# jasonppy/VoiceCraft

Measured on AMD Instinct MI355X. Metric: codec_tokens_per_sec, higher is better.
Workload: dtype bf16; 1 GPU; giga830M TTS, batch 1/GPU, Lx=80, 150 prompt frames -> 650 generated frames (16 s total), top_k=40, hipGraph=on; parallelism=dp1 (utterance-sharded, one all_gather)

## Files before the change

include/vc_engine.h:

```cpp
#ifndef VC_ENGINE_H
#define VC_ENGINE_H

#include <stdint.h>

#ifdef __cplusplus
extern "C" {
#endif

#define VC_OK 0
#define VC_EINVAL (-1)
#define VC_ESTATE (-2)
#define VC_EHIP (-3)
#define VC_ECAP (-4)
#define VC_EMISSING (-5)

#define VC_DTYPE_F32 0
#define VC_DTYPE_BF16 1
#define VC_DTYPE_I64 2

#define VC_MAX_CODEBOOKS 8
#define VC_MAX_SPANS 8
#define VC_MAX_SILENCE 8

typedef struct vc_engine vc_engine;
// ... 134 lines not shown
  void* x_out;
  int32_t dtype, H, hd, S_max, rows, nsplit, nt, fast, part16;
} vc_debug_attn_args;
int vc_debug_attn(const vc_debug_attn_args* a, void* stream);
typedef struct vc_debug_attn8_args {
  vc_debug_attn_args base;
  void* kcache8;
  void* vcache8;
  void* kvshift8;
  int32_t rps, pack;
} vc_debug_attn8_args;
int vc_debug_attn8(const vc_debug_attn8_args* a, void* stream);
int vc_kv8_quantize_host(const uint16_t* bf16_rows, int n_rows, int hd, uint8_t* codes, int8_t* shift);
int vc_box_probe(long long bytes, int hops, float res[2], void* stream);
int vc_debug_plan(const vc_model_cfg* cfg, int compute_dtype, int rows, int32_t out[16]);
int vc_debug_read(vc_engine* e, const char* name, void* host_dst, int64_t nbytes);
int vc_last_timing(const vc_engine* e, float ms[3]);
int vc_bench_kernel(vc_engine* e, const char* which, int n_rows, int iters, float* avg_ms,
                    double* alg_bytes, void* stream);

#ifdef __cplusplus
}
#endif
#endif
```

voicecraft_amd/_lib.py:

```python
from __future__ import annotations

import ctypes as C
import os
from pathlib import Path

HERE = Path(__file__).resolve().parent
LIB_PATH = HERE / "libvcengine.so"

VC_DTYPE_F32, VC_DTYPE_BF16, VC_DTYPE_I64 = 0, 1, 2
VC_MAX_SILENCE = 8


class ModelCfg(C.Structure):
    _fields_ = [(n, C.c_int32) for n in (
        "d_model", "nhead", "num_layers", "n_codebooks", "audio_vocab_size", "n_special", "text_rows",
        "head_hidden", "empty_token", "eog", "audio_pad_token", "eos", "reduced_eog", "encodec_sr",
        "max_n_spans", "max_seqs", "max_positions")]


class SampleCfg(C.Structure):
    _fields_ = [
        ("top_k", C.c_int32), ("top_p", C.c_float), ("temperature", C.c_float),
        ("stop_repetition", C.c_int32), ("n_silence", C.c_int32),
        ("silence_tokens", C.c_int32 * VC_MAX_SILENCE), ("seed", C.c_uint64),
# ... 67 lines not shown
    "vc_debug_sample": (C.c_int, [C.c_void_p, C.c_int, C.POINTER(SampleCfg), C.c_int, C.c_void_p, C.c_void_p]),
    "vc_debug_attn": (C.c_int, [C.POINTER(DebugAttnArgs), C.c_void_p]),
    "vc_debug_attn8": (C.c_int, [C.POINTER(DebugAttn8Args), C.c_void_p]),
    "vc_kv8_quantize_host": (C.c_int, [C.c_void_p, C.c_int, C.c_int, C.c_void_p, C.c_void_p]),
    "vc_edit": (C.c_int, [C.c_void_p, C.c_void_p, C.c_int, C.c_void_p, C.c_int, C.POINTER(C.c_int32), C.c_int,
                          C.POINTER(C.c_int32), C.POINTER(SampleCfg), C.c_void_p, C.c_int, C.c_void_p, C.c_int,
                          C.POINTER(C.c_int), C.c_void_p, C.c_int, C.POINTER(C.c_int), C.c_void_p]),
    "vc_edit_multi": (C.c_int, [C.c_void_p, C.c_int, C.c_void_p, C.POINTER(C.c_int32), C.c_void_p, C.POINTER(C.c_int32),
                                C.POINTER(C.c_int32), C.POINTER(C.c_int32), C.POINTER(C.c_int32), C.POINTER(SampleCfg),
                                C.c_void_p, C.c_int, C.c_void_p, C.c_int, C.POINTER(C.c_int), C.c_void_p, C.c_int,
                                C.POINTER(C.c_int), C.c_void_p]),
    "vc_pattern_shift": (C.c_int, [C.c_void_p, C.c_int, C.c_int, C.c_int, C.c_int64, C.c_void_p, C.c_void_p]),
    "vc_pattern_revert": (C.c_int, [C.c_void_p, C.c_int, C.c_int, C.c_int, C.c_int, C.c_int64, C.c_void_p, C.c_void_p]),
    "vc_pattern_unshift": (C.c_int, [C.c_void_p, C.c_int, C.c_int, C.c_void_p, C.c_void_p]),
    "vc_debug_plan": (C.c_int, [C.c_void_p, C.c_int, C.c_int, C.POINTER(C.c_int32)]),
    "vc_box_probe": (C.c_int, [C.c_longlong, C.c_int, C.POINTER(C.c_float), C.c_void_p]),
    "vc_debug_read": (C.c_int, [C.c_void_p, C.c_char_p, C.c_void_p, C.c_int64]),
    "vc_last_timing": (C.c_int, [C.c_void_p, C.POINTER(C.c_float)]),
    "vc_bench_kernel": (C.c_int, [C.c_void_p, C.c_char_p, C.c_int, C.c_int, C.POINTER(C.c_float),
                                  C.POINTER(C.c_double), C.c_void_p]),
}

_lib = None


def load() -> C.CDLL:
    global _lib
    if _lib is not None:
        return _lib
    path = Path(os.environ.get("VC_ENGINE_LIB", LIB_PATH))
# ... 29 lines not shown
```

voicecraft_amd/build.py:

```python
from __future__ import annotations

import hashlib
import os
import subprocess
import sys
from pathlib import Path

HERE = Path(__file__).resolve().parent
CSRC = HERE / "csrc"
LIB = HERE / "libvcengine.so"
SOURCES = ["vc_gemm.hip", "vc_gemm_pf.hip", "vc_gemm_wd.hip", "vc_gemm_w13.hip", "vc_gemm_w8.hip", "vc_attn.hip", "vc_tokens.hip", "vc_engine.hip", "vc_codec.hip"]
FLAGS = ["--offload-arch=gfx950", "-O3", "-std=c++17", "-fPIC", "-Wno-unused-result", "-Wno-unused-value"]


def _hipcc() -> str:
    for cand in (os.environ.get("HIPCC"), "/opt/rocm/bin/hipcc", "hipcc"):
        if cand and (os.path.isabs(cand) and os.path.exists(cand) or not os.path.isabs(cand)):
            return cand
    raise RuntimeError("hipcc not found")


def _digest(paths) -> str:
    h = hashlib.sha256()
    for p in sorted(paths):
        h.update(p.name.encode())
        h.update(p.read_bytes())
# ... 59 lines not shown
```

voicecraft_amd/csrc/vc_common.h:

```cpp
#pragma once
#include <hip/hip_runtime.h>
#include <stdint.h>
#include "../../include/vc_engine.h"

typedef __attribute__((ext_vector_type(4))) float f32x4;
typedef __attribute__((ext_vector_type(8))) __bf16 bf16x8;
typedef __attribute__((ext_vector_type(4))) unsigned int u32x4;

#define VC_ROWS 16
#define VC_MAX_SEQS 64
#ifndef VC_MAX_ROWS
#define VC_MAX_ROWS 2048
#endif
#define VC_SLAB_ROWS (VC_MAX_ROWS + 5)
#define VC_MAX_NSPLIT 8
#define VC_MAX_KSPLIT 4
#define VC_MAX_SEG 32
#ifndef VC_TH_QKV
#define VC_TH_QKV 12
#endif
#define VC_VPL 34

struct bf16_t { uint16_t u; };

// ... 354 lines not shown
hipError_t vc_launch_gemm_frp(const GemmArgs& a, int dtype, hipStream_t s);
int vc_gemm_frp_ok(int rows, int N, int K, int dtype);
hipError_t vc_launch_gemm_qp(const GemmArgs& a, int dtype, hipStream_t s);
int vc_gemm_qp_ok(int rows, int N, int K, int dtype);
enum { VC_PK_W13 = 0, VC_PK_W8 = 1, VC_PK_N = 2 };
struct vc_packed_kind {
  int group_frags, group_u4;
  int lc;
  hipError_t (*pack)(const uint4* img, long n_frags, uint4* planes, unsigned char* side, unsigned int* counts, hipStream_t s);
  hipError_t (*row)(const GemmArgs& a, const uint4* planes, const uint32_t* side, int pro, int epi, hipStream_t s);
};
const vc_packed_kind& vc_packed(int kind);
int vc_gemm_packed_fr1_ng(int kind, int N, int K, int dtype, int nw);
hipError_t vc_launch_w13_pack(const uint4* img, long n_frags, uint4* planes, unsigned char* side, unsigned int* counts, hipStream_t s);
hipError_t vc_launch_gemm_fr1_w13(const GemmArgs& a, const uint4* planes, const uint32_t* side, int pro, int epi, hipStream_t s);
hipError_t vc_launch_w8_pack(const uint4* img, long n_frags, uint4* planes, unsigned char* side, unsigned int* counts, hipStream_t s);
hipError_t vc_launch_gemm_fr1_w8(const GemmArgs& a, const uint4* planes, const uint32_t* side, int pro, int epi, hipStream_t s);
extern int vc_blk_dbg_mask;
enum { VC_LC_ROWS_GEMM = 0, VC_LC_MT2 = 1, VC_LC_MT4 = 2, VC_LC_BLK64 = 3, VC_LC_BLK128_SBS = 4, VC_LC_BLK128_2X2 = 5,
       VC_LC_BLK64_OCC2 = 6, VC_LC_LN_ROWS = 7, VC_LC_ROWS_ATTN = 8, VC_LC_TILE_ATTN = 9, VC_LC_ROWS_GEMM_FR = 10, VC_LC_BIG256 = 11, VC_LC_BIG128 = 12, VC_LC_ROW_GEMM_FR1 = 13, VC_LC_TILE_ATTN64 = 14, VC_LC_ROWS_GEMM_FRP = 15, VC_LC_WD = 16, VC_LC_ROWS_GEMM_QP = 17, VC_LC_W13 = 18, VC_LC_W8 = 19, VC_LC_KV8_ATTN = 20, VC_LC_KV8_PACK = 21, VC_LC_N = 22 };
extern long long vc_launch_counts[VC_LC_N];
hipError_t vc_launch_ln_rows(const GemmArgs& a, int dtype, hipStream_t s);
hipError_t vc_launch_attn(const AttnArgs& a, int dtype, int rows_cap, hipStream_t s);
hipError_t vc_launch_kv8_pack(const Kv8PackArgs& a, hipStream_t s);
hipError_t vc_launch_tile_attn(const AttnArgs& a, int dtype, hipStream_t s);
hipError_t vc_launch_tile_attn64(const AttnArgs& a, hipStream_t s);
hipError_t vc_launch_prompt(const PromptArgs& a, hipStream_t s);
hipError_t vc_launch_sample(const SampleArgs& a, bool grouped, hipStream_t s);
struct RepackArgs {
  SeqState* st;
  SeqState* st_fin;
  float* dec_h;
  int* row_seq;
  int* row_pos;
  int* logit_row;
// ... 92 lines not shown
```

voicecraft_amd/csrc/vc_engine.hip:

```cpp
#include <math.h>
#include <stdarg.h>
#include <stdio.h>
#include <stdlib.h>
#include <limits.h>
#include <string.h>

#include <algorithm>
#include <chrono>
#include <deque>
#include <map>
#include <string>
#include <tuple>
#include <vector>

#include "vc_common.h"

namespace {

std::string g_create_err;

struct RawTensor {
  std::vector<int64_t> shape;
  float* dev = nullptr;
  long numel = 0;
// ... 4 lines not shown
  uint4 *Wo8 = nullptr, *W28 = nullptr;
  uint4 *Wqkv16 = nullptr;
  uint4 *Wqkv8 = nullptr;
  float *bqkv = nullptr, *bo = nullptr, *b1 = nullptr, *b2 = nullptr;
  float bo_mean = 0.f, b2_mean = 0.f;
  float *wg_qkv = nullptr, *wg_1 = nullptr;
  void *kc = nullptr, *vc = nullptr;
  unsigned char *kc8 = nullptr, *vc8 = nullptr;
  signed char* sh8 = nullptr;
  struct Packed {
    uint4* planes = nullptr;
    uint32_t* side = nullptr;
    int state = 0;
    int refused = 0;
  } packed[VC_PK_N][2];
};
enum { W13_F2 = 0, W13_QKV = 1 };
constexpr int W8_BITS[2] = {1, 4};

struct Plan { int n_tiles, KT, ksplit, nchunk; };

enum { HF_ERR = 0, HF_STAGE = 1, HF_SHARE = 2, HF_ACTIVE = 8, HF_LIVE0 = 9, HF_LIVE1 = 10, HF_LIVE_STEPS = 11, HF_GATHER_N = 12 };
enum { HM_CAPTURE = 1, HM_INSTANTIATE = 2, HM_LOOP = 3, HM_SPARE = 4, HM_LAUNCHED = 5, HM_REPACKS = 6 };
enum { SS_ADMITTED = 0, SS_ADMITTED_LIVE = 1, SS_TURNS = 2, SS_WIDENINGS = 3, SS_NARROWINGS = 4, SS_LIVE_ROWS = 5, SS_LAUNCHED_ROWS = 6 };

}

struct vc_engine {
  vc_model_cfg cfg{};
  int device = 0;
// ... 54 lines not shown
  int attn_nt = 2;
  int fr_rows = VC_ROWS;
  int tile_attn = 2, tile_attn_min_rows = 768;
  int fr_one = 1;
  int fr_pair = 1;
  int qkv_p8 = 2;
  int qkv16 = 1;
  int wide_heads = 1;
  int wide_gemm = 1;
  int wd_stage = 1;
  int shrink = 1;
  bool has_fr8 = false, has_qkv8 = false, has_qkv16 = false;
  int w13 = 5;
  bool has_w13 = false;
  unsigned int* w13_counts = nullptr;
  int w8_req = 0;
  int w8 = 0;
  int kv8_req = 0;
  int kv8 = 0;
  Kv8Layer* kv8_tab = nullptr;
  int cur_rows = 0;
  int attn_fast = 1;
  int hq = 1;
  void *hqA = nullptr, *hqB = nullptr;
  float* row_mu[2] = {nullptr, nullptr};
  float* mu_zero = nullptr;
  int att_p16 = 1;
  static constexpr int attn_blocks_multi = 512, attn_blocks_one = 256;
  int prefill_rows_per_pass = VC_MAX_ROWS;
  hipEvent_t ev[3]{};
// ... 112 lines not shown
int pack_folded(vc_engine* e, const std::string& wkey, const std::string& bkey, const std::string& ln_prefix,
                int N, int Kdim, uint4** Wout, float** wg, float** cb, int th = 16) {
  const RawTensor *tw, *tb, *tg, *tbe;
  int rc;
  if ((rc = need(e, wkey, {N, Kdim}, &tw))) return rc;
  if ((rc = need(e, bkey, {N}, &tb))) return rc;
  if ((rc = need(e, ln_prefix + "weight", {Kdim}, &tg))) return rc;
  if ((rc = need(e, ln_prefix + "bias", {Kdim}, &tbe))) return rc;
  if ((rc = pack_matrix(e, wkey, N, Kdim, Wout, th, tg->dev))) return rc;
  if ((rc = dalloc(e, wg, (size_t)N))) return rc;
  if ((rc = dalloc(e, cb, (size_t)N))) return rc;
  HIPCHK(e, vc_launch_fold_vecs(tw->dev, tg->dev, tbe->dev, tb->dev, *wg, *cb, N, Kdim, e->dtype, 0));
  return VC_OK;
}

int pack_planes(vc_engine* e, Layer& ly, int kind, int which, const uint4* image, long n_frags) {
  if (!e->w13_counts) { int rc = dalloc(e, &e->w13_counts, (size_t)4); if (rc) return rc; }
  const vc_packed_kind& pk = vc_packed(kind);
  Layer::Packed& p = ly.packed[kind][which];
  const size_t mark = e->allocs.size();
  const double bytes0 = e->bytes_total;
  int rc;
  if ((rc = dalloc(e, &p.planes, (size_t)(n_frags / pk.group_frags) * pk.group_u4))) return rc;
  if ((rc = dalloc(e, &p.side, (size_t)(n_frags / 4)))) return rc;
  HIPCHK(e, pk.pack(image, n_frags, p.planes, reinterpret_cast<unsigned char*>(p.side), e->w13_counts, 0));
  unsigned int cnt[2] = {0, 0};
  HIPCHK(e, hipMemcpy(cnt, e->w13_counts, sizeof cnt, hipMemcpyDeviceToHost));
  p.refused = (int)cnt[0];
  if (cnt[0] == 0 && cnt[1] == 0) { p.state = 1; return VC_OK; }
  p.state = 2;
  while (e->allocs.size() > mark) { (void)hipFree(e->allocs.back()); e->allocs.pop_back(); }
  e->bytes_total = bytes0;
  p.planes = nullptr; p.side = nullptr;
  return VC_OK;
}

int keep_vec(vc_engine* e, const std::string& key, int n, float** out, float* mean = nullptr) {
  const RawTensor* t;
  int rc = need(e, key, {n}, &t);
  if (rc) return rc;
  rc = dalloc(e, out, (size_t)n);
  if (rc) return rc;
  HIPCHK(e, hipMemcpy(*out, t->dev, (size_t)n * 4, hipMemcpyDeviceToDevice));
  if (mean) {
    std::vector<float> host((size_t)n);
    HIPCHK(e, hipMemcpy(host.data(), t->dev, (size_t)n * 4, hipMemcpyDeviceToHost));
    double sum = 0.0;
    for (float v : host) sum += v;
    *mean = (float)(sum / n);
// ... 248 lines not shown
  GemmArgs g = base_args(e, rs, e->p_f1, 4 * d, d);
  g.Wp = ly.W1; nt_bit(e, g, NT_F1); g.bias = ly.b1; g.wg = ly.wg_1;
  g.out = e->act; g.out_ld = 4 * d; g.mt = p.mt;
  if (p.form == FORM_FR) {
    g.h_in = r.h_in;
    if (p.hq) {
      g.x_in = e->hqA; g.x_ld = d; g.row_mu = e->row_mu[1]; g.mu_shift = ly.bo_mean; g.row_mu_out = e->row_mu[0];
      HIPCHK(e, vc_launch_gemm(g, e->dtype, PRO_LNQ, EPI_RELU, 1, 1, s));
    } else {
      HIPCHK(e, vc_launch_gemm(g, e->dtype, PRO_LNW, EPI_RELU, 1, 1, s));
    }
    return VC_OK;
  }
  set_resid(e, g, r);
  if (!p.ln_launch) {
    HIPCHK(e, vc_launch_gemm(g, e->dtype, PRO_LN, EPI_RELU, 1, 1, s));
    return VC_OK;
  }
  g.x_in = e->xn; g.x_ld = d;
  if (p.wd) HIPCHK(e, vc_launch_gemm_wd(g, e->dtype, EPI_RELU, 1, 1, s));
  else HIPCHK(e, vc_launch_gemm(g, e->dtype, PRO_PLAIN, EPI_RELU, 1, 1, s));
  return VC_OK;
}

int site_ffn_down(vc_engine* e, const PassPlan& p, const RowSrc& rs, const Layer& ly, hipStream_t s) {
  const int d = e->d;
  GemmArgs g = base_args(e, rs, e->p_f2, d, 4 * d);
  g.x_in = e->act; g.x_ld = 4 * d;
  if (p.form == FORM_FR || p.fd) {
    g.Wp = ly.W28; g.bias = ly.b2;
    g.h_in = e->hA; g.h_out = e->hB;
// ... 421 lines not shown
}

int nonzero(int v) { return v ? 1 : 0; }
int two_or_one(int v) { return v == 2 ? 2 : 1; }
int low6(int v) { return v & 63; }
int whole_tiles(int v) { return v / VC_ROWS * VC_ROWS; }

struct Val { int vc_engine::*f; int lo, hi; };
struct OptDesc {
  const char *name, *env, *tag;
  Val v0;
  int (*pre)(int);
  Val v1;
  int (*check)(vc_engine*, const char* name, int v0);
  int vc_engine::*only_if;
};
using E = vc_engine;
const OptDesc OPTIONS[] = {
    {"graph_steps", "VC_GRAPH_STEPS", "g", {&E::steps_per_graph, 1, 64}},
    {"nt", "VC_NT", "nt", {&E::nt_decode, 0, 63}, low6, {&E::attn_nt, 0, 2}},
    {"finished_rows", "VC_FINISHED_ROWS", "fr", {&E::fr_rows, 0, VC_ROWS}, nullptr, {}, need_fr8},
    {"fr_pair", "VC_FR_PAIR", "fr", {&E::fr_pair, 0, 1}, nonzero},
    {"att_p16", "VC_ATT_P16", "fr", {&E::att_p16, 0, 1}, nonzero},
    {"hq", "VC_HQ", "fr", {&E::hq, 0, 1}, nonzero},
    {"tile_attn", "VC_TILE_ATTN", "ta", {&E::tile_attn, 1, 2}, two_or_one, {&E::tile_attn_min_rows, 64, INT_MAX}},
    {"fr_one", "VC_FR_ONE", "r1", {&E::fr_one, 0, 2}, nullptr, {}, need_fr8},
    {"attn_fast", "VC_ATTN_FAST", "r1", {&E::attn_fast, 0, 1}, nonzero},
    {"qkv_p8", "VC_QKV_P8", "r1", {&E::qkv_p8, 0, 2}, nullptr, {}, need_qkv8},
    {"qkv16", "VC_QKV16", "q16", {&E::qkv16, 0, 1}, nonzero, {}, need_qkv16},
    {"wide_heads", "VC_WIDE_HEADS", "q16", {&E::wide_heads, 0, 1}, nonzero},
    {"wide_gemm", "VC_WIDE_GEMM", "q16", {&E::wide_gemm, 0, 1}, nonzero},
    {"wd_stage", "VC_WD_STAGE", "q16", {&E::wd_stage, 0, 1}, nonzero},
    {"shrink", "VC_SHRINK", "sh", {&E::shrink, 0, 1}, nonzero},
    {"w13", "VC_W13", "w13", {&E::w13, 0, 5}, nullptr, {}, need_mask},
    {"w8", nullptr, "w8", {&E::w8, 0, 5}, nullptr, {}, need_w8, &E::w8_req},
    {"kv8", nullptr, "kv8", {&E::kv8, 0, 1}, nonzero, {}, need_kv8, &E::kv8_req},
    {"prefill_rows", "VC_PREFILL_ROWS", nullptr, {&E::prefill_rows_per_pass, VC_ROWS, VC_MAX_ROWS}, whole_tiles},
};

int apply_option(vc_engine* e, const std::string& name, const char* value) {
  int v[3] = {0, 0, 0};
  const int n = sscanf(value ? value : "", "%d,%d,%d", &v[0], &v[1], &v[2]);
  if (n < 1) return fail(e, VC_EINVAL, "option '%s': '%s' is not a number list", name.c_str(), value ? value : "(null)");
  for (const OptDesc& o : OPTIONS) {
    if (name != o.name) continue;
    if (o.check)
      if (const int rc = o.check(e, o.name, v[0])) return rc;
    e->*o.v0.f = std::max(o.v0.lo, std::min(o.pre ? o.pre(v[0]) : v[0], o.v0.hi));
    if (o.v1.f && n >= 2) e->*o.v1.f = std::max(o.v1.lo, std::min(v[1], o.v1.hi));
    return VC_OK;
  }
  return fail(e, VC_EINVAL, "unknown option '%s'", name.c_str());
}

void refresh_opt_state(vc_engine* e) {
  std::string& t = e->opt_state;
  t.clear();
  const char* tag = "";
  for (const OptDesc& o : OPTIONS) {
    if (!o.tag || (o.only_if && !(e->*o.only_if))) continue;
    if (strcmp(tag, o.tag)) t += std::string(t.empty() ? "" : "|") + o.tag + "=";
    else t += ",";
    tag = o.tag;
    t += std::to_string(e->*o.v0.f);
    if (o.v1.f) t += "," + std::to_string(e->*o.v1.f);
  }
}

int apply_env_presets(vc_engine* e) {
  for (const OptDesc& o : OPTIONS)
    if (const char* v = o.env ? getenv(o.env) : nullptr) {
      if (!strcmp(o.env, "VC_NT") && !strcmp(v, "1")) v = "63";
      if (const int rc = apply_option(e, o.name, v)) return rc;
    }
  refresh_opt_state(e);
// ... 24 lines not shown
  if (rows == 1) {
    out[8] = p.fd ? 1 : 0;
    out[9] = p.qkv_fr1 ? 1 : 0;
  }
  if (fr && rows <= VC_FR_MAX_ROWS) {
    out[10] = p.frp ? 1 : 0;
    out[9] = p.qp ? 2 : 0;
  }
  if (rows > VC_ROWS) {
    out[11] = p.wd ? 1 : 0;
    out[12] = wd_ksplit(&e, d, d); out[13] = wd_ksplit(&e, d, 4 * d);
    out[14] = vc_gemm_wd_kpw(d, compute_dtype, 1); out[15] = vc_gemm_wd_kpw(c->head_hidden, compute_dtype, 1);
  }
  return VC_OK;
}

extern "C" int vc_set_option(vc_engine* e, const char* name, const char* value) {
  int rc = check_idle(e);
  if (rc) return rc;
  if (!name || !value) return fail(e, VC_EINVAL, "null argument to vc_set_option");
  rc = apply_option(e, name, value);
  refresh_opt_state(e);
  return rc;
}

extern "C" const char* vc_version(void) { return "vcengine 0.1 (gfx950)"; }

extern "C" const char* vc_last_error(const vc_engine* e) { return e ? e->err.c_str() : g_create_err.c_str(); }

extern "C" int vc_create(const vc_model_cfg* c, int hip_device, vc_engine** out) {
// ... 147 lines not shown
void decide_images(vc_engine* e) {
  const int d = e->d;
  const char* env_fr = getenv("VC_FINISHED_ROWS");
  const char* env_f1 = getenv("VC_FR_ONE");
  const bool want_fr8 = !(env_fr && atoi(env_fr) == 0 && env_f1 && atoi(env_f1) == 0);
  const char* env_q16 = getenv("VC_QKV16");
  const bool want_qkv16 = env_q16 ? atoi(env_q16) != 0 : e->B_max > VC_ROWS;
  if (!want_qkv16) e->qkv16 = 0;
  const char* env_p8 = getenv("VC_QKV_P8");
  const bool want_p8 = !(env_p8 && atoi(env_p8) == 0) && !(env_f1 && atoi(env_f1) == 0);
  e->has_fr8 = want_fr8;
  e->has_qkv8 = want_fr8 && want_p8 && vc_gemm_fr1_ok(3 * d, d, e->dtype, 4);
  e->has_qkv16 = want_qkv16;
  const char* env_w13 = getenv("VC_W13");
  e->has_w13 = e->dtype == VC_DTYPE_BF16 && !(env_w13 && atoi(env_w13) == 0);
}

int pack_layer(vc_engine* e, int l) {
  const int d = e->d;
  const bool want_fr8 = e->has_fr8, want_qkv16 = e->has_qkv16;
  int rc;
  const std::string pre = "decoder.layers." + std::to_string(l) + ".";
  Layer& ly = e->layers[l];
  if ((rc = pack_folded(e, pre + "self_attn.in_proj_weight", pre + "self_attn.in_proj_bias", pre + "norm1.", 3 * d, d,
                        &ly.Wqkv, &ly.wg_qkv, &ly.bqkv, VC_TH_QKV))) return rc;
  if (want_qkv16) {
    const RawTensor* tg1;
    if ((rc = need(e, pre + "norm1.weight", {d}, &tg1))) return rc;
    if ((rc = pack_matrix(e, pre + "self_attn.in_proj_weight", 3 * d, d, &ly.Wqkv16, 16, tg1->dev))) return rc;
  }
// ... 3 lines not shown
                        &ly.W1, &ly.wg_1, &ly.b1))) return rc;
  if ((rc = pack_matrix(e, pre + "linear2.weight", d, 4 * d, &ly.W2))) return rc;
  if (want_fr8) {
    if ((rc = pack_matrix(e, pre + "self_attn.out_proj.weight", d, d, &ly.Wo8, VC_TH_RES))) return rc;
    if ((rc = pack_matrix(e, pre + "linear2.weight", d, 4 * d, &ly.W28, VC_TH_RES))) return rc;
    if (e->has_qkv8) {
      const RawTensor* tg1;
      if ((rc = need(e, pre + "norm1.weight", {d}, &tg1))) return rc;
      if ((rc = pack_matrix(e, pre + "self_attn.in_proj_weight", 3 * d, d, &ly.Wqkv8, VC_TH_RES, tg1->dev))) return rc;
    }
  }
  if ((rc = keep_vec(e, pre + "linear2.bias", d, &ly.b2, &ly.b2_mean))) return rc;
  const int pack_mask[VC_PK_N] = {e->has_w13 ? 5 : 0, e->w8_req};
  for (int kind = 0; kind < VC_PK_N; ++kind) {
    if ((pack_mask[kind] & W8_BITS[W13_F2]) && ly.W28 && vc_gemm_packed_fr1_ng(kind, d, 4 * d, e->dtype, VC_FR_WAVES) &&
        (rc = pack_planes(e, ly, kind, W13_F2, ly.W28, (long)(d / VC_TH_RES) * (4 * d / 64)))) return rc;
    if ((pack_mask[kind] & W8_BITS[W13_QKV]) && ly.Wqkv8 && vc_gemm_packed_fr1_ng(kind, 3 * d, d, e->dtype, 4) &&
        (rc = pack_planes(e, ly, kind, W13_QKV, ly.Wqkv8, (long)(3 * d / VC_TH_RES) * (d / 64)))) return rc;
  }
  const size_t cache_bytes = (size_t)e->B_max * e->H * e->S_max * e->hd * e->esz;
  if ((rc = dalloc(e, &ly.kc, cache_bytes))) return rc;
  if ((rc = dalloc(e, &ly.vc, cache_bytes))) return rc;
  if (e->kv8_req) {
    const size_t vals = (size_t)e->B_max * e->H * e->S_max * e->hd;
    if ((rc = dalloc0(e, &ly.kc8, vals, vals)) || (rc = dalloc0(e, &ly.vc8, vals, vals)) ||
        (rc = dalloc0(e, &ly.sh8, vals / e->hd * 2, vals / e->hd * 2))) return rc;
  }
  for (const char* k2 : {"self_attn.in_proj_weight", "self_attn.out_proj.weight", "linear1.weight", "linear2.weight"}) {
    auto it = e->raw.find(pre + k2);
    if (it != e->raw.end()) { HIPCHK(e, hipDeviceSynchronize()); (void)hipFree(it->second.dev); e->raw.erase(it); }
  }
  return VC_OK;
}

// ... 1618 lines not shown
  else if (n == "host_ms") { host_src = e->host_ms; avail = 8 * 8; }
  else if (n == "options") {
    memset(host_dst, 0, (size_t)nbytes);
    memcpy(host_dst, e->opt_state.c_str(), std::min<size_t>((size_t)nbytes > 0 ? (size_t)nbytes - 1 : 0, e->opt_state.size()));
    return VC_OK;
  }
  else if (n == "w13_stats" || n == "w8_stats") {
    const int kind = n == "w13_stats" ? VC_PK_W13 : VC_PK_W8;
    std::vector<int32_t> v;
    for (const Layer& ly : e->layers)
      for (int w = 0; w < 2; ++w) { v.push_back(ly.packed[kind][w].state); v.push_back(ly.packed[kind][w].refused); }
    if (nbytes > (int64_t)(v.size() * 4)) return fail(e, VC_ECAP, "debug buffer '%s' holds %lld bytes", n.c_str(), (long long)(v.size() * 4));
    memcpy(host_dst, v.data(), (size_t)nbytes);
    return VC_OK;
  }
  else if (n == "launch_counts") { host_src = vc_launch_counts; avail = VC_LC_N * 8; }
  else if (n == "stream") {
    if (!e->ts) return fail(e, VC_ESTATE, "no streaming TTS call is open (vc_tts_stream_begin)");
    if (nbytes != 3 * 4) return fail(e, VC_ECAP, "debug buffer 'stream' holds 12 bytes");
    const int32_t v[3] = {1 + e->ts->L.complete, e->ts->emitted, e->ts->L.over ? 1 : 0};
    memcpy(host_dst, v, sizeof v);
    return VC_OK;
  }
  else if (n == "session_slots") {
    if (!e->sess) return fail(e, VC_ESTATE, "no decode session is open (vc_session_open)");
    std::vector<int32_t> v{e->sess->B};
    v.insert(v.end(), e->sess->slot_ticket.begin(), e->sess->slot_ticket.end());
    if (nbytes != (int64_t)(v.size() * 4)) return fail(e, VC_ECAP, "debug buffer 'session_slots' holds %lld bytes", (long long)(v.size() * 4));
    memcpy(host_dst, v.data(), (size_t)nbytes);
    return VC_OK;
// ... 125 lines not shown
```

voicecraft_amd/engine.py:

```python
from __future__ import annotations

import ast
import ctypes as C
import logging
import math
import random
from argparse import Namespace
from typing import Iterable

import torch

from . import _lib
from ._lib import EngineError, ModelCfg, SampleCfg, check

_DTYPES = {"bf16": _lib.VC_DTYPE_BF16, "bfloat16": _lib.VC_DTYPE_BF16, torch.bfloat16: _lib.VC_DTYPE_BF16,
           "fp32": _lib.VC_DTYPE_F32, "float32": _lib.VC_DTYPE_F32, torch.float32: _lib.VC_DTYPE_F32}


def _sine_table(n: int, d: int) -> torch.Tensor:
    pos = torch.arange(0, n, dtype=torch.float32).unsqueeze(1)
    div = torch.exp(torch.arange(0, d, 2, dtype=torch.float32) * -(math.log(10000.0) / d))
    pe = torch.zeros(n, d)
    pe[:, 0::2] = torch.sin(pos * div)
    pe[:, 1::2] = torch.cos(pos * div)
# ... 554 lines not shown
        return bytes(self.debug_read("options", (256,), torch.uint8).tolist()).split(b"\0")[0].decode()

    def last_timing_ms(self):
        ms = (C.c_float * 3)()
        check(self.lib.vc_last_timing(self._h, ms), self._h, "vc_last_timing")
        return {"prefill_ms": ms[0], "decode_ms": ms[1], "total_ms": ms[2]}

    def bench_kernel(self, which: str, n_rows: int = 1, iters: int = 50):
        ms, nbytes = C.c_float(0), C.c_double(0)
        check(self.lib.vc_bench_kernel(self._h, which.encode(), n_rows, iters, C.byref(ms), C.byref(nbytes), self._stream()),
              self._h, "vc_bench_kernel")
        return ms.value, nbytes.value

    LAUNCH_FORMS = ("rows_gemm", "mt2", "mt4", "blk64", "blk128_sbs", "blk128_2x2", "blk64_occ2", "ln_rows", "rows_attn",
                    "tile_attn", "rows_gemm_fr", "big256", "big128", "row_gemm_fr1", "tile_attn64", "rows_gemm_frp", "wd", "rows_gemm_qp", "w13", "w8",
                    "kv8_attn", "kv8_pack")

    def launch_counts(self) -> dict:
        c = self.debug_read("launch_counts", (len(self.LAUNCH_FORMS),), torch.int64)
        return {n: int(c[i]) for i, n in enumerate(self.LAUNCH_FORMS)}

    W13_MATRICES = ("ffn_down", "qkv")
    W13_STATES = ("not_applicable", "packed", "refused")

    def w13_stats(self) -> list:
        L = int(self.args.num_decoder_layers)
        v = self.debug_read("w13_stats", (L, 2, 2), torch.int32).tolist()
        return [{m: {"state": self.W13_STATES[v[l][i][0]], "refused_fragments": v[l][i][1]} for i, m in enumerate(self.W13_MATRICES)}
                for l in range(L)]

    W8_MATRICES = ("ffn_down", "qkv")
    W8_MASK = 5

    def w8_stats(self) -> list:
        L = int(self.args.num_decoder_layers)
        v = self.debug_read("w8_stats", (L, 2, 2), torch.int32).tolist()
        return [{m: {"state": self.W13_STATES[v[l][i][0]], "refused_fragments": v[l][i][1]} for i, m in enumerate(self.W8_MATRICES)}
                for l in range(L)]

    def debug_read(self, name: str, shape, dtype=torch.float32) -> torch.Tensor:
        out = torch.empty(shape, dtype=dtype)
        check(self.lib.vc_debug_read(self._h, name.encode(), C.c_void_p(out.data_ptr()), out.numel() * out.element_size()),
              self._h, "vc_debug_read")
        return out
# ... 456 lines not shown
```

Before: 8004 codec-tokens/s.

## Add W13-packed single-row FFN up-projection kernel with fused LayerNorm prologue

Adds a new decode kernel for the FFN up-projection (linear1) that reads weights from the compressed W13 packed-plane format instead of dense bf16. The LayerNorm, residual-part summation and ReLU epilogue are fused in. Weights are packed at load time with norm2 folded in, and the dense image is freed afterwards. The aim is to cut HBM weight traffic for the memory-bound single-row GEMM. In exchange it adds a decode step and extra packing memory, and depends on the W13 compression being acceptable for this matrix.

```diff
diff --git a/include/vc_engine.h b/include/vc_engine.h
--- a/include/vc_engine.h
+++ b/include/vc_engine.h
@@ -172,6 +172,7 @@
 int vc_kv8_quantize_host(const uint16_t* bf16_rows, int n_rows, int hd, uint8_t* codes, int8_t* shift);
 int vc_box_probe(long long bytes, int hops, float res[2], void* stream);
 int vc_debug_plan(const vc_model_cfg* cfg, int compute_dtype, int rows, int32_t out[16]);
+int vc_debug_up13_tiles(int d_model, int compute_dtype);
 int vc_debug_read(vc_engine* e, const char* name, void* host_dst, int64_t nbytes);
 int vc_last_timing(const vc_engine* e, float ms[3]);
 int vc_bench_kernel(vc_engine* e, const char* which, int n_rows, int iters, float* avg_ms,
diff --git a/voicecraft_amd/_lib.py b/voicecraft_amd/_lib.py
--- a/voicecraft_amd/_lib.py
+++ b/voicecraft_amd/_lib.py
@@ -105,6 +105,7 @@
     "vc_pattern_revert": (C.c_int, [C.c_void_p, C.c_int, C.c_int, C.c_int, C.c_int, C.c_int64, C.c_void_p, C.c_void_p]),
     "vc_pattern_unshift": (C.c_int, [C.c_void_p, C.c_int, C.c_int, C.c_void_p, C.c_void_p]),
     "vc_debug_plan": (C.c_int, [C.c_void_p, C.c_int, C.c_int, C.POINTER(C.c_int32)]),
+    "vc_debug_up13_tiles": (C.c_int, [C.c_int, C.c_int]),
     "vc_box_probe": (C.c_int, [C.c_longlong, C.c_int, C.POINTER(C.c_float), C.c_void_p]),
     "vc_debug_read": (C.c_int, [C.c_void_p, C.c_char_p, C.c_void_p, C.c_int64]),
     "vc_last_timing": (C.c_int, [C.c_void_p, C.POINTER(C.c_float)]),
diff --git a/voicecraft_amd/build.py b/voicecraft_amd/build.py
--- a/voicecraft_amd/build.py
+++ b/voicecraft_amd/build.py
@@ -9,7 +9,7 @@
 HERE = Path(__file__).resolve().parent
 CSRC = HERE / "csrc"
 LIB = HERE / "libvcengine.so"
-SOURCES = ["vc_gemm.hip", "vc_gemm_pf.hip", "vc_gemm_wd.hip", "vc_gemm_w13.hip", "vc_gemm_w8.hip", "vc_attn.hip", "vc_tokens.hip", "vc_engine.hip", "vc_codec.hip"]
+SOURCES = ["vc_gemm.hip", "vc_gemm_pf.hip", "vc_gemm_wd.hip", "vc_gemm_w13.hip", "vc_gemm_w8.hip", "vc_gemm_up1.hip", "vc_attn.hip", "vc_tokens.hip", "vc_engine.hip", "vc_codec.hip"]
 FLAGS = ["--offload-arch=gfx950", "-O3", "-std=c++17", "-fPIC", "-Wno-unused-result", "-Wno-unused-value"]
 
 
diff --git a/voicecraft_amd/csrc/vc_common.h b/voicecraft_amd/csrc/vc_common.h
--- a/voicecraft_amd/csrc/vc_common.h
+++ b/voicecraft_amd/csrc/vc_common.h
@@ -392,11 +392,13 @@
 int vc_gemm_packed_fr1_ng(int kind, int N, int K, int dtype, int nw);
 hipError_t vc_launch_w13_pack(const uint4* img, long n_frags, uint4* planes, unsigned char* side, unsigned int* counts, hipStream_t s);
 hipError_t vc_launch_gemm_fr1_w13(const GemmArgs& a, const uint4* planes, const uint32_t* side, int pro, int epi, hipStream_t s);
+int vc_gemm_up1_ok(int d, int dtype);
+hipError_t vc_launch_gemm_up1(const GemmArgs& a, const uint4* planes, const uint32_t* side, hipStream_t s);
 hipError_t vc_launch_w8_pack(const uint4* img, long n_frags, uint4* planes, unsigned char* side, unsigned int* counts, hipStream_t s);
 hipError_t vc_launch_gemm_fr1_w8(const GemmArgs& a, const uint4* planes, const uint32_t* side, int pro, int epi, hipStream_t s);
 extern int vc_blk_dbg_mask;
 enum { VC_LC_ROWS_GEMM = 0, VC_LC_MT2 = 1, VC_LC_MT4 = 2, VC_LC_BLK64 = 3, VC_LC_BLK128_SBS = 4, VC_LC_BLK128_2X2 = 5,
-       VC_LC_BLK64_OCC2 = 6, VC_LC_LN_ROWS = 7, VC_LC_ROWS_ATTN = 8, VC_LC_TILE_ATTN = 9, VC_LC_ROWS_GEMM_FR = 10, VC_LC_BIG256 = 11, VC_LC_BIG128 = 12, VC_LC_ROW_GEMM_FR1 = 13, VC_LC_TILE_ATTN64 = 14, VC_LC_ROWS_GEMM_FRP = 15, VC_LC_WD = 16, VC_LC_ROWS_GEMM_QP = 17, VC_LC_W13 = 18, VC_LC_W8 = 19, VC_LC_KV8_ATTN = 20, VC_LC_KV8_PACK = 21, VC_LC_N = 22 };
+       VC_LC_BLK64_OCC2 = 6, VC_LC_LN_ROWS = 7, VC_LC_ROWS_ATTN = 8, VC_LC_TILE_ATTN = 9, VC_LC_ROWS_GEMM_FR = 10, VC_LC_BIG256 = 11, VC_LC_BIG128 = 12, VC_LC_ROW_GEMM_FR1 = 13, VC_LC_TILE_ATTN64 = 14, VC_LC_ROWS_GEMM_FRP = 15, VC_LC_WD = 16, VC_LC_ROWS_GEMM_QP = 17, VC_LC_W13 = 18, VC_LC_W8 = 19, VC_LC_KV8_ATTN = 20, VC_LC_KV8_PACK = 21, VC_LC_ROW_GEMM_UP1 = 22, VC_LC_N = 23 };
 extern long long vc_launch_counts[VC_LC_N];
 hipError_t vc_launch_ln_rows(const GemmArgs& a, int dtype, hipStream_t s);
 hipError_t vc_launch_attn(const AttnArgs& a, int dtype, int rows_cap, hipStream_t s);
diff --git a/voicecraft_amd/csrc/vc_engine.hip b/voicecraft_amd/csrc/vc_engine.hip
--- a/voicecraft_amd/csrc/vc_engine.hip
+++ b/voicecraft_amd/csrc/vc_engine.hip
@@ -42,6 +42,7 @@
     int state = 0;
     int refused = 0;
   } packed[VC_PK_N][2];
+  Packed up13;
 };
 enum { W13_F2 = 0, W13_QKV = 1 };
 constexpr int W8_BITS[2] = {1, 4};
@@ -126,6 +127,8 @@
   int w13 = 5;
   bool has_w13 = false;
   unsigned int* w13_counts = nullptr;
+  int up13 = 1;
+  bool has_up13 = false;
   int w8_req = 0;
   int w8 = 0;
   int kv8_req = 0;
@@ -268,10 +271,9 @@
   return VC_OK;
 }
 
-int pack_planes(vc_engine* e, Layer& ly, int kind, int which, const uint4* image, long n_frags) {
+int pack_planes(vc_engine* e, Layer::Packed& p, int kind, const uint4* image, long n_frags) {
   if (!e->w13_counts) { int rc = dalloc(e, &e->w13_counts, (size_t)4); if (rc) return rc; }
   const vc_packed_kind& pk = vc_packed(kind);
-  Layer::Packed& p = ly.packed[kind][which];
   const size_t mark = e->allocs.size();
   const double bytes0 = e->bytes_total;
   int rc;
@@ -287,6 +289,27 @@
   e->bytes_total = bytes0;
   p.planes = nullptr; p.side = nullptr;
   return VC_OK;
+}
+
+void dfree(vc_engine* e, void* p, size_t bytes) {
+  auto it = std::find(e->allocs.begin(), e->allocs.end(), p);
+  if (it == e->allocs.end()) return;
+  e->allocs.erase(it);
+  (void)hipFree(p);
+  e->bytes_total -= (double)bytes;
+}
+
+int pack_up13(vc_engine* e, Layer& ly, const std::string& pre) {
+  const int d = e->d;
+  const RawTensor* tg2;
+  uint4* img = nullptr;
+  int rc;
+  if ((rc = need(e, pre + "norm2.weight", {d}, &tg2))) return rc;
+  if ((rc = pack_matrix(e, pre + "linear1.weight", 4 * d, d, &img, VC_TH_RES, tg2->dev))) return rc;
+  const long n_frags = (long)(4 * d / VC_TH_RES) * (d / 64);
+  rc = pack_planes(e, ly.up13, VC_PK_W13, img, n_frags);
+  dfree(e, img, (size_t)n_frags * 1024);
+  return rc;
 }
 
 int keep_vec(vc_engine* e, const std::string& key, int n, float** out, float* mean = nullptr) {
@@ -565,7 +588,9 @@
   }
   set_resid(e, g, r);
   if (!p.ln_launch) {
-    HIPCHK(e, vc_launch_gemm(g, e->dtype, PRO_LN, EPI_RELU, 1, 1, s));
+    const bool up1 = p.fd && e->up13 && ly.up13.state == 1 && g.nt && r.n_parts >= 1 && r.n_parts <= 2;
+    if (up1) HIPCHK(e, vc_launch_gemm_up1(g, ly.up13.planes, ly.up13.side, s));
+    else HIPCHK(e, vc_launch_gemm(g, e->dtype, PRO_LN, EPI_RELU, 1, 1, s));
     return VC_OK;
   }
   g.x_in = e->xn; g.x_ld = d;
@@ -1017,6 +1042,7 @@
   Val v1;
   int (*check)(vc_engine*, const char* name, int v0);
   int vc_engine::*only_if;
+  int quiet_at = -1;
 };
 using E = vc_engine;
 const OptDesc OPTIONS[] = {
@@ -1038,6 +1064,7 @@
     {"w13", "VC_W13", "w13", {&E::w13, 0, 5}, nullptr, {}, need_mask},
     {"w8", nullptr, "w8", {&E::w8, 0, 5}, nullptr, {}, need_w8, &E::w8_req},
     {"kv8", nullptr, "kv8", {&E::kv8, 0, 1}, nonzero, {}, need_kv8, &E::kv8_req},
+    {"up13", "VC_UP13", "up13", {&E::up13, 0, 1}, nonzero, {}, nullptr, nullptr, 1},
     {"prefill_rows", "VC_PREFILL_ROWS", nullptr, {&E::prefill_rows_per_pass, VC_ROWS, VC_MAX_ROWS}, whole_tiles},
 };
 
@@ -1061,7 +1088,7 @@
   t.clear();
   const char* tag = "";
   for (const OptDesc& o : OPTIONS) {
-    if (!o.tag || (o.only_if && !(e->*o.only_if))) continue;
+    if (!o.tag || (o.only_if && !(e->*o.only_if)) || (o.quiet_at >= 0 && e->*o.v0.f == o.quiet_at)) continue;
     if (strcmp(tag, o.tag)) t += std::string(t.empty() ? "" : "|") + o.tag + "=";
     else t += ",";
     tag = o.tag;
@@ -1116,6 +1143,8 @@
   }
   return VC_OK;
 }
+
+extern "C" int vc_debug_up13_tiles(int d_model, int compute_dtype) { return vc_gemm_up1_ok(d_model, compute_dtype); }
 
 extern "C" int vc_set_option(vc_engine* e, const char* name, const char* value) {
   int rc = check_idle(e);
@@ -1293,6 +1322,8 @@
   e->has_qkv16 = want_qkv16;
   const char* env_w13 = getenv("VC_W13");
   e->has_w13 = e->dtype == VC_DTYPE_BF16 && !(env_w13 && atoi(env_w13) == 0);
+  const char* env_up13 = getenv("VC_UP13");
+  e->has_up13 = want_fr8 && vc_gemm_up1_ok(d, e->dtype) != 0 && !(env_up13 && atoi(env_up13) == 0);
 }
 
 int pack_layer(vc_engine* e, int l) {
@@ -1326,10 +1357,11 @@
   const int pack_mask[VC_PK_N] = {e->has_w13 ? 5 : 0, e->w8_req};
   for (int kind = 0; kind < VC_PK_N; ++kind) {
     if ((pack_mask[kind] & W8_BITS[W13_F2]) && ly.W28 && vc_gemm_packed_fr1_ng(kind, d, 4 * d, e->dtype, VC_FR_WAVES) &&
-        (rc = pack_planes(e, ly, kind, W13_F2, ly.W28, (long)(d / VC_TH_RES) * (4 * d / 64)))) return rc;
+        (rc = pack_planes(e, ly.packed[kind][W13_F2], kind, ly.W28, (long)(d / VC_TH_RES) * (4 * d / 64)))) return rc;
     if ((pack_mask[kind] & W8_BITS[W13_QKV]) && ly.Wqkv8 && vc_gemm_packed_fr1_ng(kind, 3 * d, d, e->dtype, 4) &&
-        (rc = pack_planes(e, ly, kind, W13_QKV, ly.Wqkv8, (long)(3 * d / VC_TH_RES) * (d / 64)))) return rc;
-  }
+        (rc = pack_planes(e, ly.packed[kind][W13_QKV], kind, ly.Wqkv8, (long)(3 * d / VC_TH_RES) * (d / 64)))) return rc;
+  }
+  if (e->has_up13 && (rc = pack_up13(e, ly, pre))) return rc;
   const size_t cache_bytes = (size_t)e->B_max * e->H * e->S_max * e->hd * e->esz;
   if ((rc = dalloc(e, &ly.kc, cache_bytes))) return rc;
   if ((rc = dalloc(e, &ly.vc, cache_bytes))) return rc;
@@ -2978,6 +3010,13 @@
     memcpy(host_dst, v.data(), (size_t)nbytes);
     return VC_OK;
   }
+  else if (n == "up13_stats") {
+    std::vector<int32_t> v;
+    for (const Layer& ly : e->layers) { v.push_back(ly.up13.state); v.push_back(ly.up13.refused); }
+    if (nbytes > (int64_t)(v.size() * 4)) return fail(e, VC_ECAP, "debug buffer '%s' holds %lld bytes", n.c_str(), (long long)(v.size() * 4));
+    memcpy(host_dst, v.data(), (size_t)nbytes);
+    return VC_OK;
+  }
   else if (n == "launch_counts") { host_src = vc_launch_counts; avail = VC_LC_N * 8; }
   else if (n == "stream") {
     if (!e->ts) return fail(e, VC_ESTATE, "no streaming TTS call is open (vc_tts_stream_begin)");
diff --git a/voicecraft_amd/csrc/vc_gemm_up1.hip b/voicecraft_amd/csrc/vc_gemm_up1.hip
--- /dev/null
+++ b/voicecraft_amd/csrc/vc_gemm_up1.hip
@@ -0,0 +1,194 @@
+#include "vc_gemm_fr1.h"
+#include "vc_w13.h"
+
+struct Up1Args : Fr1PackedArgs {};
+
+int vc_gemm_up1_ok(int d, int dtype) {
+  if (dtype != VC_DTYPE_BF16 || d <= 0 || d % 1024 != 0) return 0;
+  const int ng = d / 1024, tiles = 4 * d / VC_TH_RES;
+  if (ng != 1 && ng != 2) return 0;
+  return tiles % 2 == 0 ? 2 : 0;
+}
+
+template <int F>
+__device__ __forceinline__ uint4 up1_frag(const uint4& la, const uint4& lb, const uint4& nb, uint32_t sg, uint32_t sidew) {
+  const uint32_t bm1 = vc_w13_bm1((sidew >> (8 * F)) & 0xffu);
+  const uint32_t l0 = F == 0 ? la.x : F == 1 ? la.z : F == 2 ? lb.x : lb.z;
+  const uint32_t l1 = F == 0 ? la.y : F == 1 ? la.w : F == 2 ? lb.y : lb.w;
+  const uint32_t n = F == 0 ? nb.x : F == 1 ? nb.y : F == 2 ? nb.z : nb.w;
+  uint4 w;
+  vc_w13_decode_half(l0, n, sg, 2 * F, bm1, &w.x, &w.y);
+  vc_w13_decode_half(l1, n, sg, 2 * F + 1, bm1, &w.z, &w.w);
+  return w;
+}
+
+template <int NG, int T>
+__global__ __launch_bounds__(256 * T) void row_gemm_up1_w13_k(const Up1Args wa) {
+  using WT = bf16_t;
+  using Tr = WTr<WT>;
+  constexpr int NW = 4, NPW = 4 * NG, TH = VC_TH_RES, SPT = 4 * TH;
+  constexpr int D = 1024 * NG, NQ = D / 4;
+  constexpr bool ON1 = NQ > 256;
+  const GemmArgs& a = wa.g;
+  extern __shared__ __attribute__((aligned(16))) char smem[];
+  VC_KTS_DECL();
+  VC_KTS(0);
+  const int tid = threadIdx.x, lane = tid & 63;
+  const int wv = __builtin_amdgcn_readfirstlane(tid >> 6);
+  const int wave = wv & 3, tg = wv >> 2;
+  const int nt = (int)blockIdx.x * T + tg;
+  const int m = lane & 15, kg = lane >> 4;
+  char* xl = smem;
+  f32x4* red = reinterpret_cast<f32x4*>(smem + (size_t)D * sizeof(WT)) + tg * (NW * 4);
+  float* stat = reinterpret_cast<float*>(smem + (size_t)D * sizeof(WT) + (size_t)T * NW * 4 * sizeof(f32x4));
+  float* msum = stat + 8;
+  const bool pro = wv < 4;
+
+  const int c0 = tid * 4, c1 = ON1 ? (tid + 256) * 4 : 0;
+  float4 pb0 = make_float4(0.f, 0.f, 0.f, 0.f), pb1 = pb0, x0 = pb0, x1 = pb0, p00 = pb0, p01 = pb0, p10 = pb0, p11 = pb0;
+  if (pro) {
+    pb0 = *reinterpret_cast<const float4*>(a.prev_bias + c0);
+    if constexpr (ON1) pb1 = *reinterpret_cast<const float4*>(a.prev_bias + c1);
+    x0 = *reinterpret_cast<const float4*>(a.h_in + c0);
+    if constexpr (ON1) x1 = *reinterpret_cast<const float4*>(a.h_in + c1);
+    const float* s0 = a.parts;
+    const float* s1 = a.parts + (long)a.rows_cap * D;
+    p00 = *reinterpret_cast<const float4*>(s0 + c0);
+    if constexpr (ON1) p10 = *reinterpret_cast<const float4*>(s0 + c1);
+    p01 = *reinterpret_cast<const float4*>(s1 + c0);
+    if constexpr (ON1) p11 = *reinterpret_cast<const float4*>(s1 + c1);
+  }
+
+  const int wunit = (m >> 3) * SPT + kg * TH + (m & 7);
+  const long G0 = ((long)nt * NW + wave) * NG;
+  const uint4* gbase = wa.planes + G0 * VC_W13_GROUP_U4;
+  uint4 la[NG], lb[NG], nb[NG];
+  uint32_t sg[NG], sb[NG];
+  int active = 1;
+#pragma unroll
+  for (int g = 0; g < NG; ++g) {
+    const uint4* gp = gbase + g * VC_W13_GROUP_U4;
+    la[g] = __builtin_bit_cast(uint4, __builtin_nontemporal_load(reinterpret_cast<const u32x4*>(gp + wunit)));
+    lb[g] = __builtin_bit_cast(uint4, __builtin_nontemporal_load(reinterpret_cast<const u32x4*>(gp + 64 + wunit)));
+    nb[g] = __builtin_bit_cast(uint4, __builtin_nontemporal_load(reinterpret_cast<const u32x4*>(gp + 128 + wunit)));
+    sg[g] = __builtin_nontemporal_load(reinterpret_cast<const uint32_t*>(gp + 192) + wunit);
+    __builtin_amdgcn_sched_barrier(0);
+    if (g == 0) {
+#pragma unroll
+      for (int j = 0; j < NG; ++j) sb[j] = wa.side[G0 + j];
+      active = *a.n_active;
+      __builtin_amdgcn_sched_barrier(0);
+    }
+  }
+  const int nfin = nt * TH + 4 * (lane & 1);
+  const float4 eb = *reinterpret_cast<const float4*>(a.bias + nfin);
+  const float4 ewg = *reinterpret_cast<const float4*>(a.wg + nfin);
+  __builtin_amdgcn_sched_barrier(0);
+#pragma unroll
+  for (int g = 0; g < NG; ++g) asm volatile("" : "+s"(sb[g]));
+  if (active == 0) return;
+  VC_KTS(1);
+
+  if (pro) {
+    if (a.has_prev_bias != 0) {
+      x0.x += pb0.x; x0.y += pb0.y; x0.z += pb0.z; x0.w += pb0.w;
+      x1.x += pb1.x; x1.y += pb1.y; x1.z += pb1.z; x1.w += pb1.w;
+    }
+    {
+      const bool u_ = 0 < a.n_parts;
+      x0.x += u_ ? p00.x : 0.f; x0.y += u_ ? p00.y : 0.f; x0.z += u_ ? p00.z : 0.f; x0.w += u_ ? p00.w : 0.f;
+      x1.x += u_ ? p10.x : 0.f; x1.y += u_ ? p10.y : 0.f; x1.z += u_ ? p10.z : 0.f; x1.w += u_ ? p10.w : 0.f;
+    }
+    {
+      const bool u_ = 1 < a.n_parts;
+      x0.x += u_ ? p01.x : 0.f; x0.y += u_ ? p01.y : 0.f; x0.z += u_ ? p01.z : 0.f; x0.w += u_ ? p01.w : 0.f;
+      x1.x += u_ ? p11.x : 0.f; x1.y += u_ ? p11.y : 0.f; x1.z += u_ ? p11.z : 0.f; x1.w += u_ ? p11.w : 0.f;
+    }
+    if (a.h_out && blockIdx.x == 0) {
+      *reinterpret_cast<float4*>(a.h_out + c0) = x0;
+      if constexpr (ON1) *reinterpret_cast<float4*>(a.h_out + c1) = x1;
+    }
+    float t_ = ((x0.x + x0.y) + (x0.z + x0.w)) + (ON1 ? ((x1.x + x1.y) + (x1.z + x1.w)) : 0.f);
+    t_ = wave_sum(t_);
+    if (lane == 0) msum[wave] = t_;
+  }
+  __syncthreads();
+  if (pro) {
+    const float4 ms_ = *reinterpret_cast<const float4*>(msum);
+    const float mu_ = ((ms_.x + ms_.y) + (ms_.z + ms_.w)) * (1.0f / (float)D);
+    WT* xr_ = reinterpret_cast<WT*>(xl);
+    float s1_ = 0.f, s2_ = 0.f;
+    {
+      const f32x4 y_ = {x0.x - mu_, x0.y - mu_, x0.z - mu_, x0.w - mu_};
+      const f32x4 q_ = store4r(xr_ + c0, y_);
+      s1_ += (q_[0] + q_[1]) + (q_[2] + q_[3]);
+      s2_ += (q_[0] * q_[0] + q_[1] * q_[1]) + (q_[2] * q_[2] + q_[3] * q_[3]);
+    }
+    if constexpr (ON1) {
+      const f32x4 y_ = {x1.x - mu_, x1.y - mu_, x1.z - mu_, x1.w - mu_};
+      const f32x4 q_ = store4r(xr_ + c1, y_);
+      s1_ += (q_[0] + q_[1]) + (q_[2] + q_[3]);
+      s2_ += (q_[0] * q_[0] + q_[1] * q_[1]) + (q_[2] * q_[2] + q_[3] * q_[3]);
+    }
+    s1_ = wave_sum(s1_);
+    s2_ = wave_sum(s2_);
+    if (lane == 0) { stat[wave * 2] = s1_; stat[wave * 2 + 1] = s2_; }
+  }
+  VC_KTS(2);
+  __syncthreads();
+  VC_KTS(3);
+
+  f32x4 acc = {0.f, 0.f, 0.f, 0.f};
+  const char* xcol = xl + ((size_t)(m & 1) * Tr::KW + (size_t)kg * Tr::EPL) * sizeof(WT);
+#pragma unroll
+  for (int g = 0; g < NG; ++g) {
+    const int gp = NPW * wave + 4 * g;
+#define VC_UP1_STEP(F)                                                                                          \
+    {                                                                                                           \
+      const uint4 xf = *reinterpret_cast<const uint4*>(xcol + (size_t)(gp + (F)) * (2 * Tr::KW * sizeof(WT)));  \
+      const uint4 wfrag = up1_frag<F>(la[g], lb[g], nb[g], sg[g], sb[g]);                                       \
+      acc = mfma_frag(wfrag, xf, acc, (WT*)nullptr);                                                            \
+    }
+    VC_UP1_STEP(0) VC_UP1_STEP(1) VC_UP1_STEP(2) VC_UP1_STEP(3)
+#undef VC_UP1_STEP
+  }
+  VC_KTS(4);
+  if (m == (kg >> 1) && m < 2) red[wave * 4 + kg] = acc;
+  __syncthreads();
+  VC_KTS(5);
+  if (wave == 0 && lane < 2) {
+    f32x4 sum = {0.f, 0.f, 0.f, 0.f};
+#pragma unroll
+    for (int w = 0; w < NW; ++w) sum += red[w * 4 + lane] + red[w * 4 + lane + 2];
+    const float4 sa = *reinterpret_cast<const float4*>(stat), sc = *reinterpret_cast<const float4*>(stat + 4);
+    const float inv_d = 1.0f / (float)D;
+    const float mean = ((sa.x + sa.z) + (sc.x + sc.z)) * inv_d;
+    const float var = fmaxf(((sa.y + sa.w) + (sc.y + sc.w)) * inv_d - mean * mean, 0.f);
+    const float rstd = 1.0f / sqrtf(var + 1e-5f);
+    sum[0] = rstd * (sum[0] - mean * ewg.x); sum[1] = rstd * (sum[1] - mean * ewg.y);
+    sum[2] = rstd * (sum[2] - mean * ewg.z); sum[3] = rstd * (sum[3] - mean * ewg.w);
+    gemm_epilogue<WT, EPI_RELU>(a, sum, 0, nfin, 0, 0, 1, eb, -1, 0);
+  }
+  VC_KTS(6);
+  VC_KTS_FLUSH();
+}
+
+size_t vc_gemm_up1_lds_bytes(int d, int tiles) {
+  return (size_t)d * sizeof(bf16_t) + (size_t)tiles * 4 * 4 * sizeof(f32x4) + 12 * sizeof(float);
+}
+
+hipError_t vc_launch_gemm_up1(const GemmArgs& a0, const uint4* planes, const uint32_t* side, hipStream_t s) {
+  const int t = vc_gemm_up1_ok(a0.K, VC_DTYPE_BF16);
+  if (!t || a0.N != 4 * a0.K || a0.d != a0.K || a0.n_rows != 1 || a0.gather_rows || !a0.nt || !planes || !side) return hipErrorInvalidValue;
+  if (a0.n_parts < 1 || a0.n_parts > 2 || !a0.has_prev_bias) return hipErrorInvalidValue;
+  Up1Args wa;
+  wa.g = a0;
+  wa.g.n_tiles = a0.N / VC_TH_RES;
+  wa.g.KT = a0.K / 32;
+  wa.planes = planes;
+  wa.side = side;
+  void (*kern)(const Up1Args) = a0.K == 2048 ? &row_gemm_up1_w13_k<2, 2> : &row_gemm_up1_w13_k<1, 2>;
+  ++vc_launch_counts[VC_LC_ROW_GEMM_UP1];
+  hipLaunchKernelGGL(kern, dim3(wa.g.n_tiles / t), dim3(256 * t), vc_gemm_up1_lds_bytes(a0.K, t), s, wa);
+  return hipGetLastError();
+}
diff --git a/voicecraft_amd/engine.py b/voicecraft_amd/engine.py
--- a/voicecraft_amd/engine.py
+++ b/voicecraft_amd/engine.py
@@ -592,7 +592,7 @@
 
     LAUNCH_FORMS = ("rows_gemm", "mt2", "mt4", "blk64", "blk128_sbs", "blk128_2x2", "blk64_occ2", "ln_rows", "rows_attn",
                     "tile_attn", "rows_gemm_fr", "big256", "big128", "row_gemm_fr1", "tile_attn64", "rows_gemm_frp", "wd", "rows_gemm_qp", "w13", "w8",
-                    "kv8_attn", "kv8_pack")
+                    "kv8_attn", "kv8_pack", "row_gemm_up1")
 
     def launch_counts(self) -> dict:
         c = self.debug_read("launch_counts", (len(self.LAUNCH_FORMS),), torch.int64)
@@ -606,6 +606,11 @@
         v = self.debug_read("w13_stats", (L, 2, 2), torch.int32).tolist()
         return [{m: {"state": self.W13_STATES[v[l][i][0]], "refused_fragments": v[l][i][1]} for i, m in enumerate(self.W13_MATRICES)}
                 for l in range(L)]
+
+    def up13_stats(self) -> list:
+        L = int(self.args.num_decoder_layers)
+        v = self.debug_read("up13_stats", (L, 2), torch.int32).tolist()
+        return [{"state": self.W13_STATES[v[l][0]], "refused_fragments": v[l][1]} for l in range(L)]
 
     W8_MATRICES = ("ffn_down", "qkv")
     W8_MASK = 5
```

Result: no change. 8056 codec-tokens/s, median of 6 (+0.7%).
